# scrose/SVDSolver

Measured on AMD Instinct MI355X. Metric: GFLOP/s for two-stage bidiag reduction, N×N fp64, 1/2/4/8 MI355X, higher is better.
Workload: dtype f64; 1 GPU; stream of independent two-stage bidiagonal reductions 8192x8192 f64, band 32, stage 2 = reference window geometry (compat); n=8192, band=32, global_batch=10, parallelism=replicas1, pipeline=stage 2 of matrix i on a second HIP stream beside stage 1 of matrix i+1, stage2_cus=32, lanes=10, stage2_streams=5, hw_queues=19

## Files before the change

### svdsolver_amd/csrc/brd_s2win.h

```cpp
#pragma once

namespace brd {

template <typename T>
struct S2Ring {
    T *d;
    int P;
    int R;
    unsigned magic;
    __device__ __forceinline__ int slot(int r) const { return fast_mod(r, R, magic); }
    __device__ __forceinline__ T *row(int r) const { return d + slot(r) * P + 31 - r; }
};

template <typename T>
struct S2Fix {
    T sig;
    T alpha;
    T tau;
    T x31;
    T xl;
};

__device__ __forceinline__ double s2_readlane(double v, int l) {
    return __hiloint2double(__builtin_amdgcn_readlane(__double2hiint(v), l),
                            __builtin_amdgcn_readlane(__double2loint(v), l));
}
__device__ __forceinline__ float s2_readlane(float v, int l) {
    return __int_as_float(__builtin_amdgcn_readlane(__float_as_int(v), l));
}

template <typename T>
struct S2Sums {
    T q0, q1, q2, q3, g0, g1, g2, g3;
};
template <typename T>
__device__ __forceinline__ void s2_pin(S2Sums<T> &u) {
    if constexpr (sizeof(T) == 4)
        asm volatile("" : "+v"(u.q0), "+v"(u.q1), "+v"(u.q2), "+v"(u.q3), "+v"(u.g0), "+v"(u.g1), "+v"(u.g2), "+v"(u.g3));
}
template <typename T, int N>
__device__ __forceinline__ S2Sums<T> s2_sums(const T (&a)[N], const T (&x)[N]) {
    static_assert(N == 32, "b = 32 windows");
    S2Sums<T> u{x[0] * x[0], (T)0, (T)0, (T)0, (T)0, (T)0, (T)0, (T)0};
#pragma unroll
    for (int j = 1; j < N - 1; j += 4) {
        u.q1 = fma(x[j], x[j], u.q1);
        u.g1 = fma(a[j], x[j], u.g1);
        if (j + 1 < N - 1) { u.q2 = fma(x[j + 1], x[j + 1], u.q2); u.g2 = fma(a[j + 1], x[j + 1], u.g2); }
        if (j + 2 < N - 1) { u.q3 = fma(x[j + 2], x[j + 2], u.q3); u.g3 = fma(a[j + 2], x[j + 2], u.g3); }
        if (j + 3 < N - 1) { u.q0 = fma(x[j + 3], x[j + 3], u.q0); u.g0 = fma(a[j + 3], x[j + 3], u.g0); }
    }
    return u;
}
template <typename T, int N>
__device__ __forceinline__ T s2_apply(T (&a)[N], const T (&x)[N], S2Sums<T> u, S2Fix<T> &f) {
    u.q0 = fma(x[N - 1], x[N - 1], u.q0);
    const T qq = (u.q0 + u.q1) + (u.q2 + u.q3);
    const T sigp = (u.g0 + u.g1) + (u.g2 + u.g3);
    const T sig = fma(a[N - 1], x[N - 1], sigp);
    const T rn = rsq_nr(qq);
    const T nrm = qq * rn;
    const T sgn = x[0] >= (T)0 ? (T)-1 : (T)1;
    const T u1 = fma(-sgn, nrm, x[0]);
    const T alpha = rcp_nr(u1);
    const T tau = -sgn * u1 * rn;
    const T dot = fma(alpha, sig, a[0]);
    const T tda = (tau * dot) * alpha;
    a[0] = fma(-tau, dot, a[0]);
#pragma unroll
    for (int j = 1; j < N; ++j) a[j] = fma(-tda, x[j], a[j]);
    f.alpha = alpha;
    f.tau = tau;
    f.x31 = x[N - 1];
    return sigp;
}
template <typename T, int N>
__device__ __forceinline__ T s2_refl(T (&a)[N], const T (&x)[N], S2Fix<T> &f) {
    return s2_apply<T, N>(a, x, s2_sums<T, N>(a, x), f);
}

template <typename T, int N>
__device__ __forceinline__ void s2_fixup(T (&a)[N], T (&x)[N], const S2Fix<T> &f, T corner, int lane) {
    const T a0 = x[N - 1];
    const T dot = fma(f.alpha, fma(corner, f.x31, f.sig), a0);
    const T tda = (f.tau * dot) * f.alpha;
    const T p = fma(-f.tau, dot, a0);
    if (lane < 32) a[N - 1] = lane == 0 ? p : fma(-tda, f.xl, a[N - 1]);
    x[N - 1] = p;
}

struct S2Pub {
    int *prog, *front;
    int prog_v, front_v;
    __device__ __forceinline__ void publish(int lane) const {
        asm volatile("" ::: "memory");
        if (lane == 0) {
            __hip_atomic_store(front, front_v, __ATOMIC_RELAXED, __HIP_MEMORY_SCOPE_WORKGROUP);
            __hip_atomic_store(prog, prog_v, __ATOMIC_RELAXED, __HIP_MEMORY_SCOPE_WORKGROUP);
        }
    }
};

template <typename T>
__device__ __forceinline__ void s2_fixup1(T &a31, T &x31, const S2Fix<T> &f, T corner, int lane) {
    const T dot = fma(f.alpha, fma(corner, f.x31, f.sig), x31);
    const T tda = (f.tau * dot) * f.alpha;
    const T p = fma(-f.tau, dot, x31);
    if (lane < 32) a31 = lane == 0 ? p : fma(-tda, f.xl, a31);
    x31 = p;
}

template <typename T, bool FULL, bool LAG2>
__device__ __forceinline__ void s2_right_w1(const S2Ring<T> &rg, int i1, int j1, int nr, int nc, int lane,
                                            bool fix, const S2Fix<T> &fi, bool defer, S2Fix<T> &fo,
                                            const S2Pub &pub) {
    constexpr int N = 32;
    const bool rok = FULL || lane < nr;
    const T *px = rg.row(i1) + j1;
    T *pa = rg.row(i1 + (rok ? lane : 0)) + j1;
    T a[N], x[N];
#pragma unroll
    for (int j = 0; j < N; ++j) {
        const bool cok = FULL || j < nc;
        x[j] = cok ? px[j] : (T)0;
        a[j] = (cok && rok) ? pa[j] : (T)0;
    }
    if (LAG2) fo.xl = px[lane & 31];
    const T corner = LAG2 ? rg.row(i1 + 31)[j1 + 31] : (T)0;
    S2Sums<T> u = s2_sums<T, N>(a, x);
    s2_pin(u);
    if (LAG2 && fix) {
        s2_fixup1<T>(a[N - 1], x[N - 1], fi, corner, lane);
        if (lane < 32) pa[N - 1] = a[N - 1];
        pub.publish(lane);
    }
    const T sigp = s2_apply<T, N>(a, x, u, fo);
    if (LAG2 && defer) {
        fo.sig = s2_readlane(sigp, 63);
        if ((lane & 31) == 31) fo.xl = x[N - 1];
    }
    if (rok && !(LAG2 && defer && lane == 63)) {
#pragma unroll
        for (int j = 0; j < N; ++j)
            if (FULL || j < nc) pa[j] = a[j];
    }
}

template <typename T, bool FULL, bool LAG2>
__device__ __forceinline__ void s2_left_w1(const S2Ring<T> &rg, int i1, int j1, int nr, int nc, int lane,
                                           bool fix, const S2Fix<T> &fi, bool defer, S2Fix<T> &fo,
                                           const S2Pub &pub) {
    constexpr int N = 32;
    const bool cok = FULL || lane < nc;
    const int q = cok ? lane : 0;
    const int s0 = rg.slot(i1);
    T a[N], x[N];
    if (LAG2) fo.xl = rg.row(i1 + (lane & 31))[j1];
    auto finish = [&](T *e31, T corner, auto store) {
        S2Sums<T> u = s2_sums<T, N>(a, x);
        s2_pin(u);
        if (LAG2 && fix) {
            s2_fixup1<T>(a[N - 1], x[N - 1], fi, corner, lane);
            if (lane < 32) *e31 = a[N - 1];
            pub.publish(lane);
        }
        const T sigp = s2_apply<T, N>(a, x, u, fo);
        if (LAG2 && defer) {
            fo.sig = s2_readlane(sigp, 63);
            if ((lane & 31) == 31) fo.xl = x[N - 1];
        }
        if (cok && !(LAG2 && defer && lane == 63)) store();
    };
    if (s0 + N <= rg.R) {
        T *bx = rg.d + s0 * rg.P + 31 + (j1 - i1);
#pragma unroll
        for (int j = 0; j < N; ++j) {
            const bool rk = FULL || j < nr;
            x[j] = rk ? bx[j * (rg.P - 1)] : (T)0;
            a[j] = (rk && cok) ? bx[j * (rg.P - 1) + q] : (T)0;
        }
        T *b31 = bx + (N - 1) * (rg.P - 1);
        finish(b31 + q, LAG2 ? b31[31] : (T)0, [&]() {
#pragma unroll
            for (int j = 0; j < N; ++j)
                if (FULL || j < nr) bx[j * (rg.P - 1) + q] = a[j];
        });
    } else {
        T *rows[N];
        int s = s0;
#pragma unroll
        for (int j = 0; j < N; ++j) {
            rows[j] = rg.d + s * rg.P + 31 + (j1 - i1) - j;
            s = s + 1 == rg.R ? 0 : s + 1;
            const bool rk = FULL || j < nr;
            x[j] = rk ? rows[j][0] : (T)0;
            a[j] = (rk && cok) ? rows[j][q] : (T)0;
        }
        finish(rows[N - 1] + q, LAG2 ? rows[N - 1][31] : (T)0, [&]() {
#pragma unroll
            for (int j = 0; j < N; ++j)
                if (FULL || j < nr) rows[j][q] = a[j];
        });
    }
}


}
```

### svdsolver_amd/csrc/brd_stage2.hip

```cpp
#include "brd_internal.h"

#include <algorithm>
#include <cstdlib>

namespace brd {

template <typename T>
__device__ __forceinline__ T ld_c(const T *p) {
    return __hip_atomic_load(p, __ATOMIC_RELAXED, __HIP_MEMORY_SCOPE_AGENT);
}
template <typename T>
__device__ __forceinline__ void st_c(T *p, T v) {
    __hip_atomic_store(p, v, __ATOMIC_RELAXED, __HIP_MEMORY_SCOPE_AGENT);
}

__device__ __forceinline__ void wave_sync2() {
    __builtin_amdgcn_fence(__ATOMIC_RELEASE, "wavefront");
    __builtin_amdgcn_wave_barrier();
    __builtin_amdgcn_fence(__ATOMIC_ACQUIRE, "wavefront");
}

template <typename T>
struct Refl {
    T alpha;
    T tau;
};

template <typename T, bool EXACT>
__device__ __forceinline__ Refl<T> refl_regs(const T (&x)[32], int L) {
    T acc = (T)0;
    double s;
    T nrm;
    if constexpr (EXACT) {
#pragma clang fp contract(off)
#pragma unroll
        for (int r = 0; r < 32; ++r)
            if (r < L) acc = acc + x[r] * x[r];
        nrm = (T)sqrt((double)acc);
        s = -copysign(1.0, (double)x[0]);
    } else {
        T acc1 = (T)0;
#pragma unroll
        for (int r = 0; r < 32; r += 2) {
            if (r < L) acc = fma(x[r], x[r], acc);
            if (r + 1 < L) acc1 = fma(x[r + 1], x[r + 1], acc1);
        }
        nrm = sqrt(acc + acc1);
        s = x[0] >= (T)0 ? -1.0 : 1.0;
    }
    const double u1 = (double)x[0] - s * (double)nrm;
    Refl<T> h;
    h.alpha = (T)(1. / u1);
    h.tau = (T)(-s * u1 / (double)nrm);
    return h;
}

template <typename T, bool EXACT>
struct WaveLds {
    T w[64];
    T h[2];
};
template <typename T>
struct WaveLds<T, true> {
    T w[64];
    T h[2];
    T x[64];
    T H[32 * 33];
    T buf[64 * 33];
};

template <typename T>
struct HbmAcc {
    T *A;
    long lda;
    __device__ __forceinline__ T *row(int r) const { return A + (long)r * lda; }
    __device__ __forceinline__ T ld(const T *p) const { return ld_c(p); }
    __device__ __forceinline__ void st(T *p, T v) const { st_c(p, v); }
};
__device__ __forceinline__ int fast_mod(int r, int R, unsigned magic) {
    int s = r - (int)__umulhi((unsigned)r, magic) * R;
    return s >= R ? s - R : s;
}

template <typename T>
struct RingAcc {
    T *d;
// ... 570 lines not shown
struct SweepFlags {
    int prog[12];
    int front[12];
    int loaded;
    int freed;
    int avail;
    int wturn;
    int wclaim;
    int wpub;
};

#ifdef BRD_S2TRACE
constexpr int kTrB0 = 600, kTrNB = 4, kTrTasks = 600, kTrPub = 1024;
struct S2Trace {
    unsigned long long task[kTrNB][12][kTrTasks][4];
    unsigned long long pub[kTrNB][8][kTrPub][2];
    int npub[kTrNB][8];
    unsigned long long bundle[kTrNB][4];
    unsigned long long wr[kTrNB][256][8];
};
__device__ S2Trace g_s2tr;
#define TRB(beta) ((beta) >= kTrB0 && (beta) < kTrB0 + kTrNB)
#define TRT(beta, w, t, k)                                                                      \
    do {                                                                                        \
        if (TRB(beta) && (t) < kTrTasks && lane == 0)                                           \
            g_s2tr.task[(beta) - kTrB0][w][t][k] = __builtin_amdgcn_s_memrealtime();            \
    } while (0)
#define TRP(beta, kind, val)                                                                    \
    do {                                                                                        \
        if (TRB(beta) && lane == 0) {                                                           \
            const int q_ = g_s2tr.npub[(beta) - kTrB0][kind]++;                                 \
            if (q_ < kTrPub) {                                                                  \
                g_s2tr.pub[(beta) - kTrB0][kind][q_][0] = __builtin_amdgcn_s_memrealtime();     \
                g_s2tr.pub[(beta) - kTrB0][kind][q_][1] = (val);                                \
            }                                                                                   \
        }                                                                                       \
    } while (0)
#define TRW(beta, q, k)                                                                         \
    do {                                                                                        \
        if (TRB(beta) && (q) < 256 && lane == 0)                                                \
            g_s2tr.wr[(beta) - kTrB0][q][k] = __builtin_amdgcn_s_memrealtime();                 \
    } while (0)
#else
#define TRT(beta, w, t, k) do {} while (0)
#define TRP(beta, kind, val) do {} while (0)
#define TRW(beta, q, k) do {} while (0)
#endif

template <typename T> constexpr int sweeps_max_threads() { return sizeof(T) == 8 ? 512 : 768; }

__device__ __forceinline__ int lds_ld(const int *p) {
    return __hip_atomic_load(p, __ATOMIC_RELAXED, __HIP_MEMORY_SCOPE_WORKGROUP);
}
__device__ __forceinline__ void lds_st(int *p, int v) {
    __hip_atomic_store(p, v, __ATOMIC_RELAXED, __HIP_MEMORY_SCOPE_WORKGROUP);
}

struct SweepStages {
    int nst;
    int B[5];
    int G[4];
};
__device__ __forceinline__ int sweeps_next(const SweepStages &st, int w, int beta, int nbundles) {
    int k = 0;
    while (k + 1 < st.nst && beta >= st.B[k + 1]) ++k;
    int nx = beta + st.G[k];
    while (k + 1 < st.nst && nx >= st.B[k + 1]) {
        ++k;
        if (w >= st.G[k]) return nbundles;
        const int b0 = st.B[k];
        nx = b0 + (((w - b0) % st.G[k]) + st.G[k]) % st.G[k];
    }
    return nx;
}
__device__ __forceinline__ int sweeps_first(const SweepStages &st, int w, int nbundles) {
    for (int k = 0; k < st.nst; ++k) {
        if (w >= st.G[k]) return nbundles;
        const int b0 = st.B[k];
        const int c = b0 + (((w - b0) % st.G[k]) + st.G[k]) % st.G[k];
        if (c < st.B[k + 1]) return c;
    }
    return nbundles;
}
template <typename T, int WR>
__global__ void __launch_bounds__(sweeps_max_threads<T>())
k_sweeps(T *A, int n, long lda, int sigma, int S, int R, unsigned magic, int *rows_done, int *err, SweepStages st)
{
    constexpr int b = 32;
    extern __shared__ __align__(16) unsigned char smem[];
    const int P = ring_pitch<T>(b);
    T *ring = (T *)smem;
    const size_t ring_bytes = ((size_t)R * P * sizeof(T) + 15) & ~(size_t)15;
    SweepFlags *F = (SweepFlags *)(smem + ring_bytes);
    const int wave = __builtin_amdgcn_readfirstlane(threadIdx.x >> 6), lane = threadIdx.x & 63;
    const S2Ring<T> rg{ring, P, R, magic};
    const int nbundles = (n - 1 + S - 1) / S;

    for (int beta = sweeps_first(st, (int)blockIdx.x, nbundles); beta < nbundles;
         beta = sweeps_next(st, (int)blockIdx.x, beta, nbundles)) {
        const int i0 = beta * S;
        const int nsw = min(S, n - 1 - i0);
        if (threadIdx.x < 12) {
            F->prog[threadIdx.x] = 0;
            F->front[threadIdx.x] = (int)threadIdx.x < nsw ? i0 + (int)threadIdx.x : n;
        }
        if (threadIdx.x == 0) {
            F->loaded = i0; F->freed = i0; F->avail = 0;
            F->wturn = 0; F->wclaim = i0; F->wpub = i0;
        }
#ifdef BRD_S2TRACE
        if (threadIdx.x == 0 && TRB(beta)) {
            g_s2tr.bundle[beta - kTrB0][0] = __builtin_amdgcn_s_memrealtime();
            g_s2tr.bundle[beta - kTrB0][2] = blockIdx.x;
            g_s2tr.bundle[beta - kTrB0][3] = __builtin_amdgcn_s_getreg((20 << 0) | (0 << 6) | (3 << 11));
        }
#endif
        __syncthreads();

        if (wave < nsw) {
            const int i = i0 + wave;
            SweepIter it;
            it.init(n, n, b, i, sigma);
            const int prev_ntask = wave > 0 ? sweep_ntask(n, n, b, i - 1, sigma) : 0;
            S2Fix<T> fx{(T)0, (T)0, (T)0, (T)0, (T)0};
            bool pend = false;
            for (int t = 0; t < it.ntask; ++t) {
                bool right;
                const Win w = it.task(t, right);
                const int nr = w.i2 - w.i1, nc = w.j2 - w.j1;
                const bool live = nr > 0 && nc > 0;
                const bool full = live && (right ? (nr == 2 * b && nc == b) : (nr == b && nc == 2 * b));
                const bool defer = kS2Lag2 && full && it.next_at_least(t, b);
                int spins = 0;
                TRT(beta, wave, t, 0);
                if (wave > 0) {
                    const int need = min(t + (defer ? 4 - BRD_S2_DEFER_LAG2 : 4), prev_ntask);
                    while (lds_ld(&F->prog[wave - 1]) < need) {
                        __builtin_amdgcn_s_sleep(0);
                        if (++spins > kSpinLimit) { if (lane == 0) st_c(err, 12); break; }
                    }
                }
                TRT(beta, wave, t, 1);
                if (live) {
                    while (lds_ld(&F->loaded) < w.i2) {
                        __builtin_amdgcn_s_sleep(0);
                        if (++spins > kSpinLimit) { if (lane == 0) st_c(err, 13); break; }
                    }
                    TRT(beta, wave, t, 2);
                    asm volatile("" ::: "memory");
                    const S2Pub pub{&F->prog[wave], &F->front[wave], t, w.i1};
                    S2Fix<T> fo;
                    if (right) {
                        if (full) s2_right_w1<T, true, kS2Lag2>(rg, w.i1, w.j1, nr, nc, lane, pend, fx, defer, fo, pub);
                        else      s2_right_w1<T, false, kS2Lag2>(rg, w.i1, w.j1, nr, nc, lane, pend, fx, defer, fo, pub);
                    } else {
                        if (full) s2_left_w1<T, true, kS2Lag2>(rg, w.i1, w.j1, nr, nc, lane, pend, fx, defer, fo, pub);
                        else      s2_left_w1<T, false, kS2Lag2>(rg, w.i1, w.j1, nr, nc, lane, pend, fx, defer, fo, pub);
                    }
                    if (defer) fx = fo;
                    asm volatile("" ::: "memory");
                }
                pend = defer;
                TRT(beta, wave, t, 3);
                if (lane == 0) {
                    lds_st(&F->front[wave], it.next_top(t));
                    if (!defer) lds_st(&F->prog[wave], t + 1);
                }
            }
        } else if (wave == S) {
            const int row_q = P * (int)sizeof(T) / 16;
            const bool ql = lane < row_q;
            const unsigned row_bytes = (unsigned)(P * (int)sizeof(T));
            const unsigned ring_lds = (unsigned)(uintptr_t)ring;
            const unsigned ring_end = ring_lds + (unsigned)R * row_bytes;
            const int dma_hi = (int)(((long)(n - 1) * lda + n + (b - 1) - P) / (lda + 1));
            int ra = i0, rl = i0, spins = 0;
            unsigned dst = ring_lds + (unsigned)rg.slot(i0) * row_bytes;
            const char *src = (const char *)(A + (long)i0 * lda + i0 - (b - 1)) + 16 * lane;
            const long rstep = (lda + 1) * (long)sizeof(T);
            const bool dma_lane = lane < row_q;
            while (rl < n) {
                const int av = lds_ld(&F->avail);
                const int fr = lds_ld(&F->freed);
                const int lim = __builtin_amdgcn_readfirstlane(min(min(av, fr + R), min(n, rl + kFly)));
                bool moved = false;
                if (ra < lim) {
                    if (ra >= 1 && ra <= dma_hi) {
                        const int k = min(lim, dma_hi + 1) - ra;
                        if (dma_lane) {
                            const char *p = src;
                            unsigned d = dst;
                            for (int q = 0; q < k; ++q) {
                                dma16_sc1(p, d);
                                p += rstep;
                                d += row_bytes;
                                if (d == ring_end) d = ring_lds;
                            }
                        }
                        src += (long)k * rstep;
                        dst += (unsigned)k * row_bytes;
                        if (dst >= ring_end) dst -= ring_end - ring_lds;
                        ra += k;
                        moved = true;
                        TRP(beta, 5, ra);
                        TRP(beta, 7, (av <= fr + R ? 0 : 1) + (lim == rl + kFly ? 2 : 0));
                    } else if (ra == rl) {
                        load_edge_row<T>(A, lda, n, b, ra, (T *)((char *)ring + (dst - ring_lds)), row_q, lane);
                        asm volatile("s_waitcnt vmcnt(0) lgkmcnt(0)" ::: "memory");
                        ++ra;
                        rl = ra;
                        src += rstep;
                        dst += row_bytes;
                        if (dst == ring_end) dst = ring_lds;
                        if (lane == 0) lds_st(&F->loaded, rl);
                        moved = true;
                    }
                }
                if (ra > rl) {
                    const int keep = max(0, ra - rl - kChunk);
                    wait_vmcnt(keep);
                    rl = ra - keep;
                    if (lane == 0) lds_st(&F->loaded, rl);
                    TRP(beta, 0, rl);
                    spins = 0;
                } else if (BRD_S2_REGLOAD && !moved && ra < av && fr + R <= ra && ra >= 1 && ra <= dma_hi) {
                    const int k = __builtin_amdgcn_readfirstlane(min(min(kRG<T>, av - ra), dma_hi + 1 - ra));
                    u32x4 g[kRG<T>];
                    {
                        const __amdgpu_buffer_rsrc_t rs = __builtin_amdgcn_make_buffer_rsrc(
                            (void *)(A + (long)ra * lda + ra - (b - 1)), (short)0, 0x7fffffff, 0x00020000);
                        const int vo = 16 * (ql ? lane : 0);
#pragma unroll
                        for (int kk = 0; kk < kRG<T>; ++kk)
                            g[kk] = __builtin_amdgcn_raw_buffer_load_b128(rs, vo, (unsigned)((kk < k ? kk : 0) * rstep), 16);
                    }
                    const int sl0 = (int)((dst - ring_lds) / row_bytes);
                    int fl = fr + R;
#pragma unroll
                    for (int kk = 0; kk < kRG<T>; ++kk) {
                        if (kk < k) {
                            const int r = ra + kk;
                            if (r >= fl) {
                                if (kk > 0 && lane == 0) lds_st(&F->loaded, r);
                                int f2 = __builtin_amdgcn_readfirstlane(lds_ld(&F->freed));
                                while (f2 + R <= r) {
                                    __builtin_amdgcn_s_sleep(0);
                                    if (++spins > kSpinLimit) { if (lane == 0) st_c(err, 14); break; }
                                    f2 = __builtin_amdgcn_readfirstlane(lds_ld(&F->freed));
                                }
                                fl = f2 + R;
                            }
                            const int sl = sl0 + kk >= R ? sl0 + kk - R : sl0 + kk;
                            if (ql) *((u32x4 *)(ring + sl * P) + lane) = g[kk];
                        }
                    }
                    ra += k;
                    rl = ra;
                    src += (long)k * rstep;
                    dst += (unsigned)k * row_bytes;
                    if (dst >= ring_end) dst -= ring_end - ring_lds;
                    if (lane == 0) lds_st(&F->loaded, rl);
                    TRP(beta, 0, rl);
                    spins = 0;
                } else if (!moved) {
                    __builtin_amdgcn_s_sleep(0);
                    if (++spins > kSpinLimit) { if (lane == 0) st_c(err, 14); break; }
                }
            }
            asm volatile("s_waitcnt vmcnt(0)" ::: "memory");
        } else if (wave == S + 1 + kSweepWriters) {
            if (beta == 0) {
                if (lane == 0) lds_st(&F->avail, n);
            } else {
                const int *done_prev = rows_done + beta - 1;
                int av = 0, spins = 0;
                while (av < n) {
                    const int v = __builtin_amdgcn_readfirstlane(ld_c(done_prev));
                    if (v != av) {
                        av = v;
                        if (lane == 0) lds_st(&F->avail, v);
                        TRP(beta, 2, v);
                        spins = 0;
                    } else {
                        __builtin_amdgcn_s_sleep(1);
                        if (++spins > kSpinLimit) { if (lane == 0) st_c(err, 16); break; }
                    }
                }
            }
        } else if (wave > S && wave <= S + kSweepWriters) {
            const int wi = wave - S - 1;
            const int row_q = P * (int)sizeof(T) / 16;
            const long gstep = (lda + 1) * (long)sizeof(T);
            for (int q = wi;; q += kSweepWriters) {
                int spins = 0;
                while (lds_ld(&F->wturn) != q) {
                    __builtin_amdgcn_s_sleep(0);
                    if (++spins > kSpinLimit) { if (lane == 0) st_c(err, 15); break; }
                }
                const int wb = __builtin_amdgcn_readfirstlane(lds_ld(&F->wclaim));
                if (wb >= n) {
                    if (lane == 0) lds_st(&F->wturn, q + 1);
                    break;
                }
                int wt = wb;
                spins = 0;
                for (;;) {
                    int fmin = n;
                    for (int s = 0; s < nsw; ++s) fmin = min(fmin, lds_ld(&F->front[s]));
                    wt = __builtin_amdgcn_readfirstlane(min(min(fmin, lds_ld(&F->loaded)), wb + WR));
                    if (wt > wb) break;
                    __builtin_amdgcn_s_sleep(0);
                    if (++spins > kSpinLimit) { if (lane == 0) st_c(err, 15); break; }
                }
                if (wt <= wb) break;
                if (lane == 0) {
                    lds_st(&F->wclaim, wt);
                    lds_st(&F->wturn, q + 1);
                }
                TRP(beta, 3, wb);
                TRW(beta, q, 0);
                const int k = wt - wb;
                constexpr int kH = WR / 2;
                const int sl0 = rg.slot(wb);
                const unsigned rstride = (unsigned)gstep;
                for (int r0 = 0; r0 < k; r0 += kH) {
                    const int kh = min(kH, k - r0);
                    const int sl = sl0 + r0 >= R ? sl0 + r0 - R : sl0 + r0;
                    const int rb = wb + r0;
                    const bool fast = kh == kH && sl + kH <= R && rb >= b - 1 && rb + kH - 1 - (b - 1) + P <= n;
                    if (fast) {
                        u32x4 v[kH];
                        const u32x4 *srow = (const u32x4 *)(ring + sl * P) + (lane < row_q ? lane : 0);
#pragma unroll
                        for (int rr = 0; rr < kH; ++rr) v[rr] = srow[rr * (P / kEpp<T>)];
                        asm volatile("s_waitcnt lgkmcnt(0)" ::: "memory");
                        TRW(beta, q, 1 + 3 * (r0 / kH));
                        spins = 0;
                        while (lds_ld(&F->freed) != rb) {
                            __builtin_amdgcn_s_sleep(0);
                            if (++spins > kSpinLimit) { if (lane == 0) st_c(err, 15); break; }
                        }
                        if (lane == 0) lds_st(&F->freed, rb + kH);
                        TRP(beta, 6, rb + kH);
                        TRW(beta, q, 2 + 3 * (r0 / kH));
                        if (lane < row_q) {
                            const __amdgpu_buffer_rsrc_t rs = __builtin_amdgcn_make_buffer_rsrc(
                                (void *)(A + (long)rb * lda + rb - (b - 1)), (short)0, 0x7fffffff, 0x00020000);
#pragma unroll
                            for (int rr = 0; rr < kH; ++rr)
                                __builtin_amdgcn_raw_buffer_store_b128(v[rr], rs, 16 * lane, rr * rstride, 16);
                        }
                        TRW(beta, q, 3 + 3 * (r0 / kH));
                    } else {
                        for (int rr = 0; rr < kh; ++rr) {
                            const int r = rb + rr;
                            const int sk = sl + rr >= R ? sl + rr - R : sl + rr;
                            const u32x4 vr = ((const u32x4 *)(ring + sk * P))[lane < row_q ? lane : 0];
                            asm volatile("s_waitcnt lgkmcnt(0)" ::: "memory");
                            if (lane < row_q) {
                                if (r >= b - 1 && r - (b - 1) + P <= n) {
                                    st16_sc1((void *)((const char *)(A + (long)r * lda + r - (b - 1)) + 16 * lane), vr);
                                } else {
                                    T *ge = A + (long)r * lda + r - (b - 1) + lane * kEpp<T>;
                                    const int cc0 = r - (b - 1) + lane * kEpp<T>;
                                    T e[kEpp<T>];
                                    __builtin_memcpy(e, &vr, 16);
#pragma unroll
                                    for (int kk = 0; kk < kEpp<T>; ++kk)
                                        if (cc0 + kk >= 0 && cc0 + kk < n) st_c(ge + kk, e[kk]);
                                }
                            }
                        }
                        spins = 0;
                        while (lds_ld(&F->freed) != rb) {
                            __builtin_amdgcn_s_sleep(0);
                            if (++spins > kSpinLimit) { if (lane == 0) st_c(err, 15); break; }
                        }
                        if (lane == 0) lds_st(&F->freed, rb + kh);
                        TRP(beta, 6, rb + kh);
                    }
                }
                TRP(beta, 4, wt);
                asm volatile("s_waitcnt vmcnt(0)" ::: "memory");
                TRW(beta, q, 7);
                spins = 0;
                while (lds_ld(&F->wpub) != wb) {
                    __builtin_amdgcn_s_sleep(0);
                    if (++spins > kSpinLimit) { if (lane == 0) st_c(err, 15); break; }
                }
                if (lane == 0) {
                    st_c(rows_done + beta, wt);
                    lds_st(&F->wpub, wt);
                }
                TRP(beta, 1, wt);
            }
        }
        __syncthreads();
#ifdef BRD_S2TRACE
        if (threadIdx.x == 0 && TRB(beta)) g_s2tr.bundle[beta - kTrB0][1] = __builtin_amdgcn_s_memrealtime();
#endif
    }
}

#ifdef BRD_S2TRACE
extern "C" int brd_dbg_s2trace(void *dst, size_t bytes, int reset) {
    if (reset) {
        static S2Trace z;
        return (int)hipMemcpyToSymbol(HIP_SYMBOL(g_s2tr), &z, sizeof(S2Trace));
    }
    return (int)hipMemcpyFromSymbol(dst, HIP_SYMBOL(g_s2tr), bytes < sizeof(S2Trace) ? bytes : sizeof(S2Trace));
}
#endif

template <typename T>
__global__ void k_extract(const T *A, int n, long lda, T *d, T *e)
{
    const int i = blockIdx.x * blockDim.x + threadIdx.x;
    if (i < n) d[i] = A[(long)i * lda + i];
    if (i < n - 1) e[i] = A[(long)i * lda + i + 1];
}

int ring_min_rows(int b, int S) { return ((3 * (S - 1)) / 2 + 2) * b + S + 8; }

template <typename T, bool EXACT>
static size_t bundle_lds_bytes(int b, int S, int R) {
    const size_t ring = ((size_t)R * ring_pitch<T>(b) * sizeof(T) + 15) & ~(size_t)15;
    return ring + (size_t)S * sizeof(WaveLds<T, EXACT>) + sizeof(BundleFlags);
}

template <typename T, bool EXACT>
static bool bundle_plan(int n, int b, int &S, int &R) {
    const size_t budget = 160 * 1024 - 512;
    static const char *senv = getenv("BRD_S2_SWEEPS");
    int smax = EXACT ? 2 : bundle_max_threads<T>() / 64 - 3;
    if (senv && atoi(senv) > 0) smax = std::min(smax, atoi(senv));
    const bool forced = senv && atoi(senv) > 0;
    for (int slack : {forced ? 8 : 16, 8}) {
        for (S = std::min(smax, std::max(1, n - 1)); S >= 1; --S) {
            const int rmin = ring_min_rows(b, S) + slack;
            if (bundle_lds_bytes<T, EXACT>(b, S, rmin) <= budget) {
                static const char *renv = getenv("BRD_S2_RING");
                const int rcap = renv && atoi(renv) > 0 ? std::max(rmin, atoi(renv)) : 1 << 30;
                R = rmin;
                while (R < n + 1 && R + 8 <= rcap && bundle_lds_bytes<T, EXACT>(b, S, R + 8) <= budget) R += 8;
                return true;
            }
        }
    }
    return false;
}

constexpr int kSweepSlack = 40;
template <typename T>
static size_t sweeps_lds_bytes(int R, int S) {
    (void)S;
    return (((size_t)R * ring_pitch<T>(32) * sizeof(T) + 15) & ~(size_t)15) + ((sizeof(SweepFlags) + 15) & ~(size_t)15);
}
template <typename T>
static bool sweeps_plan(int n, int &S, int &R) {
    const size_t budget = 160 * 1024;
    static const char *senv = getenv("BRD_S2_SWEEPS");
    int smax = sweeps_max_threads<T>() / 64 - 2 - kSweepWriters;
    if (smax > 12) smax = 12;
    if (senv && atoi(senv) > 0) smax = std::min(smax, atoi(senv));
    for (S = std::min(smax, std::max(1, n - 1)); S >= 1; --S) {
        const int rmin = ring_min_rows(32, S) + kSweepSlack;
        if (sweeps_lds_bytes<T>(rmin, S) <= budget) {
            R = rmin;
            while (R < n + 1 && sweeps_lds_bytes<T>(R + 1, S) <= budget) ++R;
            return true;
        }
    }
    return false;
}

static int coresident_limit(const void *fn, int threads, size_t lds) {
    int per_cu = 0, dev = 0, cus = 0;
    if (hipOccupancyMaxActiveBlocksPerMultiprocessor(&per_cu, fn, threads, lds) != hipSuccess) return 0;
    hipGetDevice(&dev);
    if (hipDeviceGetAttribute(&cus, hipDeviceAttributeMultiprocessorCount, dev) != hipSuccess) return 0;
    return per_cu * cus;
}

static SweepStages sweep_stages(int n, int S, int nbundles, int grid) {
    SweepStages st{};
    st.nst = 1;
    st.B[0] = 0;
    st.G[0] = grid;
    st.B[1] = nbundles;
    const char *e = getenv("BRD_S2_STAGES");
    if (e && atoi(e) == 0) return st;
    int g = grid;
    for (int beta = 0; beta < nbundles && st.nst < 4; ++beta) {
        const double alive = (double)(n - beta * S) / (64.0 * S) + 1.0;
        const int half = g / 2;
        if (half >= kStageMin && g % 2 == 0 && beta >= st.B[st.nst - 1] + g &&
            alive * kStageMargin + kStageSpare <= half) {
            st.B[st.nst] = beta;
            st.G[st.nst] = half;
            ++st.nst;
            g = half;
        }
    }
    st.B[st.nst] = nbundles;
    return st;
}

template <typename T>
hipError_t launch_band2bd(T *A, int n, long lda, int b, bool exact_order, bool sigma_geom, int *prog, int *err,
                          int nwaves, hipStream_t s)
{
    hipError_t e = hipMemsetAsync(prog, 0, sizeof(int) * (size_t)(n + 1), s);
    if (e != hipSuccess) return e;
    const int sg = sigma_geom ? 1 : 0;
    static const char *sel = getenv("BRD_S2_SCHEDULE");
    const bool pipe = sel && sel[0] == 'p';
    int S = 0, R = 0;
    const bool fast32 = !exact_order && b == 32;
    if (!pipe && fast32 && n >= 64 && sweeps_plan<T>(n, S, R)) {
        const int nbundles = (n - 1 + S - 1) / S;
        const dim3 block(64 * (S + 2 + kSweepWriters));
        const unsigned magic = (unsigned)((0x100000000ull + R - 1) / R);
        const bool w32 = sweep_rows_for(n) == 32;
        const void *fn = w32 ? (const void *)k_sweeps<T, 32> : (const void *)k_sweeps<T, 16>;
        const size_t lds = sweeps_lds_bytes<T>(R, S);
        e = hipFuncSetAttribute(fn, hipFuncAttributeMaxDynamicSharedMemorySize, (int)lds);
        if (e != hipSuccess) return e;
        const int cap = coresident_limit(fn, (int)block.x, lds);
        if (cap < 1) return hipErrorInvalidConfiguration;
        const int grid = std::max(1, std::min(std::min(nwaves, cap), nbundles));
        const SweepStages st = sweep_stages(n, S, nbundles, grid);
        if (w32) hipLaunchKernelGGL((k_sweeps<T, 32>), dim3(grid), block, lds, s, A, n, lda, sg, S, R, magic, prog, err, st);
        else     hipLaunchKernelGGL((k_sweeps<T, 16>), dim3(grid), block, lds, s, A, n, lda, sg, S, R, magic, prog, err, st);
        return hipGetLastError();
    }
    const bool ok = exact_order ? bundle_plan<T, true>(n, b, S, R) : bundle_plan<T, false>(n, b, S, R);
    if (!pipe && ok && n >= 64) {
        const int nbundles = (n - 1 + S - 1) / S;
        const dim3 block(64 * (S + 3));
        const unsigned magic = (unsigned)((0x100000000ull + R - 1) / R);
        const void *fn = exact_order ? (const void *)k_band2bd_bundle<T, true> : (const void *)k_band2bd_bundle<T, false>;
        const size_t lds = exact_order ? bundle_lds_bytes<T, true>(b, S, R) : bundle_lds_bytes<T, false>(b, S, R);
        e = hipFuncSetAttribute(fn, hipFuncAttributeMaxDynamicSharedMemorySize, (int)lds);
        if (e != hipSuccess) return e;
        const int cap = coresident_limit(fn, (int)block.x, lds);
        if (cap < 1) return hipErrorInvalidConfiguration;
        const int grid = std::max(1, std::min(std::min(nwaves, cap), nbundles));
        if (exact_order)
            hipLaunchKernelGGL((k_band2bd_bundle<T, true>), dim3(grid), block, lds, s, A, n, lda, b, sg, S, R, magic, prog, err);
        else
            hipLaunchKernelGGL((k_band2bd_bundle<T, false>), dim3(grid), block, lds, s, A, n, lda, b, sg, S, R, magic, prog, err);
        return hipGetLastError();
    }
    const void *pfn = exact_order ? (const void *)k_band2bd_pipe<T, true> : (const void *)k_band2bd_pipe<T, false>;
    const int cap = coresident_limit(pfn, 64, 0);
    if (cap < 1) return hipErrorInvalidConfiguration;
    const int grid = std::max(1, std::min(std::min(nwaves, cap), n - 1));
    if (exact_order)
        hipLaunchKernelGGL((k_band2bd_pipe<T, true>), dim3(grid), dim3(64), 0, s, A, n, n, lda, b, sg, prog, err);
    else
        hipLaunchKernelGGL((k_band2bd_pipe<T, false>), dim3(grid), dim3(64), 0, s, A, n, n, lda, b, sg, prog, err);
    return hipGetLastError();
}

template <typename T>
hipError_t launch_extract_bidiag(const T *A, int n, long lda, T *d, T *e, hipStream_t s)
{
    hipLaunchKernelGGL((k_extract<T>), dim3((n + 255) / 256), dim3(256), 0, s, A, n, lda, d, e);
    return hipGetLastError();
}

template hipError_t launch_band2bd<double>(double *, int, long, int, bool, bool, int *, int *, int, hipStream_t);
template hipError_t launch_band2bd<float>(float *, int, long, int, bool, bool, int *, int *, int, hipStream_t);
template hipError_t launch_extract_bidiag<double>(const double *, int, long, double *, double *, hipStream_t);
template hipError_t launch_extract_bidiag<float>(const float *, int, long, float *, float *, hipStream_t);

}
```

Before: 27710 GFLOP/s.

## Store stage-2 sweep ring in LDS with per-phase narrow row pitch

Adds a phase-dependent narrow row layout for the fp64 stage-2 LDS ring. Each row stores only the columns its phase in the 32-row group actually touches, so the same LDS budget holds more rows. The loader, writer and left-window code are rewritten to use per-phase offsets and widths, and the sweep index is made a compile-time constant per wave. The layout is on by default for fp64 and caps sweeps per bundle at 4 (default 3) instead of up to 12, so parallelism within a bundle drops. It also adds more complex index arithmetic.

After: 19450 GFLOP/s. -29.8%, worse.

```diff
diff --git a/svdsolver_amd/csrc/brd_s2_ring.h b/svdsolver_amd/csrc/brd_s2_ring.h
--- /dev/null
+++ b/svdsolver_amd/csrc/brd_s2_ring.h
@@ -0,0 +1,81 @@
+#pragma once
+
+#include <cstddef>
+
+#ifndef BRD_HD
+#ifdef __HIPCC__
+#define BRD_HD __host__ __device__
+#else
+#define BRD_HD
+#endif
+#endif
+
+namespace brd {
+namespace s2ring {
+
+constexpr int kB = 32;
+constexpr int kMaxSweeps = 4;
+constexpr int kWidePhases = kMaxSweeps - 1;
+constexpr int kWideW = 96;
+constexpr int kWideLo = -31;
+constexpr int kNarrowW = 68;
+
+BRD_HD constexpr int ph_width(int p) { return p < kWidePhases ? kWideW : kNarrowW; }
+BRD_HD constexpr int ph_skew(int p) { return p < 16 ? 1 : 0; }
+BRD_HD constexpr int ph_dlo(int p) { return p < kWidePhases ? kWideLo : -p - ph_skew(p); }
+BRD_HD constexpr int ph_off(int p) {
+    return p < kWidePhases ? kWideW * p : kWideW * kWidePhases + kNarrowW * (p - kWidePhases) + 2 * (p >> 3);
+}
+BRD_HD constexpr int ph_zero(int p) { return ph_off(p) - ph_dlo(p); }
+constexpr int kGroupElems = ph_off(31) + kNarrowW;
+
+BRD_HD constexpr int idx_off(int idx) { return (idx >> 5) * kGroupElems + ph_off(idx & 31); }
+
+BRD_HD inline int ring_index(int i0, int r, int R) {
+    int u = (r - i0 - 1) % R;
+    return u < 0 ? u + R : u;
+}
+
+struct Row {
+    int off;
+    int c0;
+    int w;
+};
+BRD_HD inline Row row_map(int i0, int r, int R) {
+    const int idx = ring_index(i0, r, R);
+    const int p = idx & 31;
+    return Row{idx_off(idx), r + ph_dlo(p), ph_width(p)};
+}
+
+BRD_HD constexpr int left_carry(int sw, int j) { return (sw + j) >> 5; }
+BRD_HD constexpr int left_off(int sw, int j) { return ph_zero((sw + j) & 31) - j; }
+
+BRD_HD constexpr int ring_min_rows(int b, int S) { return ((3 * (S - 1)) / 2 + 2) * b + S + 8; }
+constexpr int kSweepSlack = 40;
+
+BRD_HD constexpr size_t ring_bytes(int groups, size_t esz) { return (size_t)groups * kGroupElems * esz; }
+
+constexpr int kDefaultSweeps = 3;
+struct Plan {
+    bool ok;
+    int S, G, R;
+    size_t bytes;
+};
+BRD_HD inline Plan plan(int n, int s_req, size_t esz, size_t budget, size_t tail) {
+    Plan pl{false, 0, 0, 0, 0};
+    int S = s_req > 0 ? s_req : kDefaultSweeps;
+    if (S > kMaxSweeps) S = kMaxSweeps;
+    if (S > n - 1) S = n - 1 > 1 ? n - 1 : 1;
+    if (budget < tail) return pl;
+    const int G = (int)((budget - tail) / ring_bytes(1, esz));
+    for (; S >= 1; --S) {
+        if (32 * G >= ring_min_rows(kB, S) + kSweepSlack) {
+            pl = Plan{true, S, G, 32 * G, ring_bytes(G, esz) + tail};
+            return pl;
+        }
+    }
+    return pl;
+}
+
+}
+}
diff --git a/svdsolver_amd/csrc/brd_s2win.h b/svdsolver_amd/csrc/brd_s2win.h
--- a/svdsolver_amd/csrc/brd_s2win.h
+++ b/svdsolver_amd/csrc/brd_s2win.h
@@ -1,15 +1,32 @@
 #pragma once
 
+#include "brd_s2_ring.h"
+
 namespace brd {
 
 template <typename T>
 struct S2Ring {
+    static constexpr bool kNarrow = false;
     T *d;
     int P;
     int R;
     unsigned magic;
     __device__ __forceinline__ int slot(int r) const { return fast_mod(r, R, magic); }
     __device__ __forceinline__ T *row(int r) const { return d + slot(r) * P + 31 - r; }
+};
+
+template <typename T>
+struct S2RingN {
+    static constexpr bool kNarrow = true;
+    T *d;
+    int R;
+    unsigned magic;
+    int org;
+    __device__ __forceinline__ int index(int r) const { return fast_mod(r - org, R, magic); }
+    __device__ __forceinline__ T *row(int r) const {
+        const int idx = index(r);
+        return d + ((idx >> 5) * s2ring::kGroupElems + s2ring::ph_zero(idx & 31)) - r;
+    }
 };
 
 template <typename T>
@@ -110,8 +127,8 @@
     x31 = p;
 }
 
-template <typename T, bool FULL, bool LAG2>
-__device__ __forceinline__ void s2_right_w1(const S2Ring<T> &rg, int i1, int j1, int nr, int nc, int lane,
+template <typename T, bool FULL, bool LAG2, typename RG>
+__device__ __forceinline__ void s2_right_w1(const RG &rg, int i1, int j1, int nr, int nc, int lane,
                                             bool fix, const S2Fix<T> &fi, bool defer, S2Fix<T> &fo,
                                             const S2Pub &pub) {
     constexpr int N = 32;
@@ -146,14 +163,13 @@
     }
 }
 
-template <typename T, bool FULL, bool LAG2>
-__device__ __forceinline__ void s2_left_w1(const S2Ring<T> &rg, int i1, int j1, int nr, int nc, int lane,
+template <typename T, bool FULL, bool LAG2, int SW, typename RG>
+__device__ __forceinline__ void s2_left_w1(const RG &rg, int i1, int j1, int nr, int nc, int lane,
                                            bool fix, const S2Fix<T> &fi, bool defer, S2Fix<T> &fo,
                                            const S2Pub &pub) {
     constexpr int N = 32;
     const bool cok = FULL || lane < nc;
     const int q = cok ? lane : 0;
-    const int s0 = rg.slot(i1);
     T a[N], x[N];
     if (LAG2) fo.xl = rg.row(i1 + (lane & 31))[j1];
     auto finish = [&](T *e31, T corner, auto store) {
@@ -171,7 +187,24 @@
         }
         if (cok && !(LAG2 && defer && lane == 63)) store();
     };
-    if (s0 + N <= rg.R) {
+    if constexpr (RG::kNarrow) {
+        const int g0 = __builtin_amdgcn_readfirstlane(rg.index(i1) >> 5);
+        const int g1 = g0 + 1 == (rg.R >> 5) ? 0 : g0 + 1;
+        T *const bg[2] = {rg.d + g0 * s2ring::kGroupElems + (j1 - i1), rg.d + g1 * s2ring::kGroupElems + (j1 - i1)};
+#pragma unroll
+        for (int j = 0; j < N; ++j) {
+            const bool rk = FULL || j < nr;
+            T *bj = bg[s2ring::left_carry(SW, j)] + s2ring::left_off(SW, j);
+            x[j] = rk ? bj[0] : (T)0;
+            a[j] = (rk && cok) ? bj[q] : (T)0;
+        }
+        T *b31 = bg[s2ring::left_carry(SW, N - 1)] + s2ring::left_off(SW, N - 1);
+        finish(b31 + q, LAG2 ? b31[31] : (T)0, [&]() {
+#pragma unroll
+            for (int j = 0; j < N; ++j)
+                if (FULL || j < nr) bg[s2ring::left_carry(SW, j)][s2ring::left_off(SW, j) + q] = a[j];
+        });
+    } else if (const int s0 = rg.slot(i1); s0 + N <= rg.R) {
         T *bx = rg.d + s0 * rg.P + 31 + (j1 - i1);
 #pragma unroll
         for (int j = 0; j < N; ++j) {
@@ -187,7 +220,7 @@
         });
     } else {
         T *rows[N];
-        int s = s0;
+        int s = rg.slot(i1);
 #pragma unroll
         for (int j = 0; j < N; ++j) {
             rows[j] = rg.d + s * rg.P + 31 + (j1 - i1) - j;
diff --git a/svdsolver_amd/csrc/brd_stage2.hip b/svdsolver_amd/csrc/brd_stage2.hip
--- a/svdsolver_amd/csrc/brd_stage2.hip
+++ b/svdsolver_amd/csrc/brd_stage2.hip
@@ -2,6 +2,7 @@
 
 #include <algorithm>
 #include <cstdlib>
+#include <type_traits>
 
 namespace brd {
 
@@ -738,24 +739,45 @@
     }
     return nbundles;
 }
-template <typename T, int WR>
+template <typename T, bool NARROW> struct SweepRing { typedef S2Ring<T> type; };
+template <typename T> struct SweepRing<T, true> { typedef S2RingN<T> type; };
+template <typename T>
+__device__ __forceinline__ void load_edge_row_n(const T *A, long lda, int n, int r, int c0, T *dst, int npc, int lane) {
+    if (lane < npc) {
+        T e[kEpp<T>];
+#pragma unroll
+        for (int k = 0; k < kEpp<T>; ++k) {
+            const int c = c0 + lane * kEpp<T> + k;
+            e[k] = (c >= 0 && c < n) ? ld_c(A + (long)r * lda + c) : (T)0;
+        }
+        u32x4 v;
+        __builtin_memcpy(&v, e, 16);
+        *(u32x4 *)(dst + lane * kEpp<T>) = v;
+    }
+}
+
+template <typename T, int WR, bool NARROW>
 __global__ void __launch_bounds__(sweeps_max_threads<T>())
 k_sweeps(T *A, int n, long lda, int sigma, int S, int R, unsigned magic, int *rows_done, int *err, SweepStages st)
 {
     constexpr int b = 32;
+    static_assert(!NARROW || sizeof(T) == 8, "the row-phase pitch is fp64 only");
     extern __shared__ __align__(16) unsigned char smem[];
     const int P = ring_pitch<T>(b);
     T *ring = (T *)smem;
-    const size_t ring_bytes = ((size_t)R * P * sizeof(T) + 15) & ~(size_t)15;
+    const size_t ring_bytes = NARROW ? s2ring::ring_bytes(R >> 5, sizeof(T))
+                                     : (((size_t)R * P * sizeof(T) + 15) & ~(size_t)15);
     SweepFlags *F = (SweepFlags *)(smem + ring_bytes);
     const int wave = __builtin_amdgcn_readfirstlane(threadIdx.x >> 6), lane = threadIdx.x & 63;
-    const S2Ring<T> rg{ring, P, R, magic};
     const int nbundles = (n - 1 + S - 1) / S;
 
     for (int beta = sweeps_first(st, (int)blockIdx.x, nbundles); beta < nbundles;
          beta = sweeps_next(st, (int)blockIdx.x, beta, nbundles)) {
         const int i0 = beta * S;
         const int nsw = min(S, n - 1 - i0);
+        typename SweepRing<T, NARROW>::type rg;
+        if constexpr (NARROW) rg = S2RingN<T>{ring, R, magic, i0 + 1 - R};
+        else                  rg = S2Ring<T>{ring, P, R, magic};
         if (threadIdx.x < 12) {
             F->prog[threadIdx.x] = 0;
             F->front[threadIdx.x] = (int)threadIdx.x < nsw ? i0 + (int)threadIdx.x : n;
@@ -810,8 +832,22 @@
                         if (full) s2_right_w1<T, true, kS2Lag2>(rg, w.i1, w.j1, nr, nc, lane, pend, fx, defer, fo, pub);
                         else      s2_right_w1<T, false, kS2Lag2>(rg, w.i1, w.j1, nr, nc, lane, pend, fx, defer, fo, pub);
                     } else {
-                        if (full) s2_left_w1<T, true, kS2Lag2>(rg, w.i1, w.j1, nr, nc, lane, pend, fx, defer, fo, pub);
-                        else      s2_left_w1<T, false, kS2Lag2>(rg, w.i1, w.j1, nr, nc, lane, pend, fx, defer, fo, pub);
+                        auto left = [&](auto swc) {
+                            constexpr int SW = decltype(swc)::value;
+                            if (full) s2_left_w1<T, true, kS2Lag2, SW>(rg, w.i1, w.j1, nr, nc, lane, pend, fx, defer, fo, pub);
+                            else      s2_left_w1<T, false, kS2Lag2, SW>(rg, w.i1, w.j1, nr, nc, lane, pend, fx, defer, fo, pub);
+                        };
+                        if constexpr (NARROW) {
+                            static_assert(s2ring::kMaxSweeps == 4, "one case per sweep of a bundle");
+                            switch (wave) {
+                                case 0: left(std::integral_constant<int, 0>{}); break;
+                                case 1: left(std::integral_constant<int, 1>{}); break;
+                                case 2: left(std::integral_constant<int, 2>{}); break;
+                                default: left(std::integral_constant<int, 3>{}); break;
+                            }
+                        } else {
+                            left(std::integral_constant<int, 0>{});
+                        }
                     }
                     if (defer) fx = fo;
                     asm volatile("" ::: "memory");
@@ -824,6 +860,107 @@
                 }
             }
         } else if (wave == S) {
+            if constexpr (NARROW) {
+            constexpr int kE = kEpp<T>;
+            const unsigned ring_lds = (unsigned)(uintptr_t)ring;
+            const int dma_hi = (int)(((long)(n - 1) * lda + n - (s2ring::kWideLo + s2ring::kWideW)) / (lda + 1));
+            int ra = i0, rl = i0, spins = 0;
+            int ia = __builtin_amdgcn_readfirstlane(rg.index(i0));
+            const char *src = (const char *)(A + (long)i0 * lda + i0) + 16 * lane;
+            const long rstep = (lda + 1) * (long)sizeof(T);
+            while (rl < n) {
+                const int av = lds_ld(&F->avail);
+                const int fr = lds_ld(&F->freed);
+                const int lim = __builtin_amdgcn_readfirstlane(min(min(av, fr + R), min(n, rl + kFly)));
+                bool moved = false;
+                if (ra < lim) {
+                    if (ra >= 1 && ra <= dma_hi) {
+                        const int k = min(lim, dma_hi + 1) - ra;
+                        const char *p = src;
+                        int ix = ia;
+                        for (int q = 0; q < k; ++q) {
+                            const int ph = ix & 31;
+                            const unsigned d = __builtin_amdgcn_readfirstlane(
+                                ring_lds + (unsigned)(s2ring::idx_off(ix) * (int)sizeof(T)));
+                            if (lane < s2ring::ph_width(ph) / kE) dma16_sc1(p + s2ring::ph_dlo(ph) * (int)sizeof(T), d);
+                            p += rstep;
+                            ix = ix + 1 == R ? 0 : ix + 1;
+                        }
+                        src += (long)k * rstep;
+                        ia = ia + k >= R ? ia + k - R : ia + k;
+                        ra += k;
+                        moved = true;
+                        TRP(beta, 5, ra);
+                        TRP(beta, 7, (av <= fr + R ? 0 : 1) + (lim == rl + kFly ? 2 : 0));
+                    } else if (ra == rl) {
+                        const int ph = ia & 31;
+                        load_edge_row_n<T>(A, lda, n, ra, ra + s2ring::ph_dlo(ph), ring + s2ring::idx_off(ia),
+                                           s2ring::ph_width(ph) / kE, lane);
+                        asm volatile("s_waitcnt vmcnt(0) lgkmcnt(0)" ::: "memory");
+                        ++ra;
+                        rl = ra;
+                        src += rstep;
+                        ia = ia + 1 == R ? 0 : ia + 1;
+                        if (lane == 0) lds_st(&F->loaded, rl);
+                        moved = true;
+                    }
+                }
+                if (ra > rl) {
+                    const int keep = max(0, ra - rl - kChunk);
+                    wait_vmcnt(keep);
+                    rl = ra - keep;
+                    if (lane == 0) lds_st(&F->loaded, rl);
+                    TRP(beta, 0, rl);
+                    spins = 0;
+                } else if (BRD_S2_REGLOAD && !moved && ra < av && fr + R <= ra && ra >= 1 && ra <= dma_hi) {
+                    const int k = __builtin_amdgcn_readfirstlane(min(min(kRG<T>, av - ra), dma_hi + 1 - ra));
+                    u32x4 g[kRG<T>];
+                    {
+                        const __amdgpu_buffer_rsrc_t rs = __builtin_amdgcn_make_buffer_rsrc(
+                            (void *)(A + (long)ra * lda + ra + s2ring::kWideLo), (short)0, 0x7fffffff, 0x00020000);
+#pragma unroll
+                        for (int kk = 0; kk < kRG<T>; ++kk) {
+                            const int kq = kk < k ? kk : 0;
+                            const int ix = ia + kq >= R ? ia + kq - R : ia + kq;
+                            const int ph = ix & 31;
+                            const int vo = 16 * (lane < s2ring::ph_width(ph) / kE ? lane : 0);
+                            g[kk] = __builtin_amdgcn_raw_buffer_load_b128(
+                                rs, vo, (unsigned)(kq * rstep + (s2ring::ph_dlo(ph) - s2ring::kWideLo) * (int)sizeof(T)), 16);
+                        }
+                    }
+                    int fl = fr + R;
+#pragma unroll
+                    for (int kk = 0; kk < kRG<T>; ++kk) {
+                        if (kk < k) {
+                            const int r = ra + kk;
+                            if (r >= fl) {
+                                if (kk > 0 && lane == 0) lds_st(&F->loaded, r);
+                                int f2 = __builtin_amdgcn_readfirstlane(lds_ld(&F->freed));
+                                while (f2 + R <= r) {
+                                    __builtin_amdgcn_s_sleep(0);
+                                    if (++spins > kSpinLimit) { if (lane == 0) st_c(err, 14); break; }
+                                    f2 = __builtin_amdgcn_readfirstlane(lds_ld(&F->freed));
+                                }
+                                fl = f2 + R;
+                            }
+                            const int ix = ia + kk >= R ? ia + kk - R : ia + kk;
+                            if (lane < s2ring::ph_width(ix & 31) / kE) *((u32x4 *)(ring + s2ring::idx_off(ix)) + lane) = g[kk];
+                        }
+                    }
+                    ra += k;
+                    rl = ra;
+                    src += (long)k * rstep;
+                    ia = ia + k >= R ? ia + k - R : ia + k;
+                    if (lane == 0) lds_st(&F->loaded, rl);
+                    TRP(beta, 0, rl);
+                    spins = 0;
+                } else if (!moved) {
+                    __builtin_amdgcn_s_sleep(0);
+                    if (++spins > kSpinLimit) { if (lane == 0) st_c(err, 14); break; }
+                }
+            }
+            asm volatile("s_waitcnt vmcnt(0)" ::: "memory");
+            } else {
             const int row_q = P * (int)sizeof(T) / 16;
             const bool ql = lane < row_q;
             const unsigned row_bytes = (unsigned)(P * (int)sizeof(T));
@@ -924,6 +1061,7 @@
                 }
             }
             asm volatile("s_waitcnt vmcnt(0)" ::: "memory");
+            }
         } else if (wave == S + 1 + kSweepWriters) {
             if (beta == 0) {
                 if (lane == 0) lds_st(&F->avail, n);
@@ -977,8 +1115,82 @@
                 TRW(beta, q, 0);
                 const int k = wt - wb;
                 constexpr int kH = WR / 2;
+                const unsigned rstride = (unsigned)gstep;
+                if constexpr (NARROW) {
+                constexpr int kE = kEpp<T>;
+                const int ix0 = __builtin_amdgcn_readfirstlane(rg.index(wb));
+                for (int r0 = 0; r0 < k; r0 += kH) {
+                    const int kh = min(kH, k - r0);
+                    const int ixb = ix0 + r0 >= R ? ix0 + r0 - R : ix0 + r0;
+                    const int rb = wb + r0;
+                    const bool fast = kh == kH && rb >= -s2ring::kWideLo &&
+                                      rb + kH - 1 + s2ring::kWideLo + s2ring::kWideW <= n;
+                    if (fast) {
+                        u32x4 v[kH];
+#pragma unroll
+                        for (int rr = 0; rr < kH; ++rr) {
+                            const int ix = ixb + rr >= R ? ixb + rr - R : ixb + rr;
+                            const int npc = s2ring::ph_width(ix & 31) / kE;
+                            v[rr] = ((const u32x4 *)(ring + s2ring::idx_off(ix)))[lane < npc ? lane : 0];
+                        }
+                        asm volatile("s_waitcnt lgkmcnt(0)" ::: "memory");
+                        TRW(beta, q, 1 + 3 * (r0 / kH));
+                        spins = 0;
+                        while (lds_ld(&F->freed) != rb) {
+                            __builtin_amdgcn_s_sleep(0);
+                            if (++spins > kSpinLimit) { if (lane == 0) st_c(err, 15); break; }
+                        }
+                        if (lane == 0) lds_st(&F->freed, rb + kH);
+                        TRP(beta, 6, rb + kH);
+                        TRW(beta, q, 2 + 3 * (r0 / kH));
+                        {
+                            const __amdgpu_buffer_rsrc_t rs = __builtin_amdgcn_make_buffer_rsrc(
+                                (void *)(A + (long)rb * lda + rb + s2ring::kWideLo), (short)0, 0x7fffffff, 0x00020000);
+#pragma unroll
+                            for (int rr = 0; rr < kH; ++rr) {
+                                const int ix = ixb + rr >= R ? ixb + rr - R : ixb + rr;
+                                const int ph = ix & 31;
+                                if (lane < s2ring::ph_width(ph) / kE)
+                                    __builtin_amdgcn_raw_buffer_store_b128(
+                                        v[rr], rs, 16 * lane,
+                                        rr * rstride + (unsigned)((s2ring::ph_dlo(ph) - s2ring::kWideLo) * (int)sizeof(T)), 16);
+                            }
+                        }
+                        TRW(beta, q, 3 + 3 * (r0 / kH));
+                    } else {
+                        for (int rr = 0; rr < kh; ++rr) {
+                            const int r = rb + rr;
+                            const int ix = ixb + rr >= R ? ixb + rr - R : ixb + rr;
+                            const int ph = ix & 31;
+                            const int npc = s2ring::ph_width(ph) / kE;
+                            const int c0 = r + s2ring::ph_dlo(ph);
+                            const u32x4 vr = ((const u32x4 *)(ring + s2ring::idx_off(ix)))[lane < npc ? lane : 0];
+                            asm volatile("s_waitcnt lgkmcnt(0)" ::: "memory");
+                            if (lane < npc) {
+                                if (c0 >= 0 && c0 + npc * kE <= n) {
+                                    st16_sc1((void *)((const char *)(A + (long)r * lda + c0) + 16 * lane), vr);
+                                } else {
+                                    T *ge = A + (long)r * lda + c0 + lane * kE;
+                                    const int cc0 = c0 + lane * kE;
+                                    T e[kE];
+                                    __builtin_memcpy(e, &vr, 16);
+#pragma unroll
+                                    for (int kk = 0; kk < kE; ++kk)
+                                        if (cc0 + kk >= 0 && cc0 + kk < n) st_c(ge + kk, e[kk]);
+                                }
+                            }
+                        }
+                        spins = 0;
+                        while (lds_ld(&F->freed) != rb) {
+                            __builtin_amdgcn_s_sleep(0);
+                            if (++spins > kSpinLimit) { if (lane == 0) st_c(err, 15); break; }
+                        }
+                        if (lane == 0) lds_st(&F->freed, rb + kh);
+                        TRP(beta, 6, rb + kh);
+                    }
+                }
+                } else {
                 const int sl0 = rg.slot(wb);
-                const unsigned rstride = (unsigned)gstep;
                 for (int r0 = 0; r0 < k; r0 += kH) {
                     const int kh = min(kH, k - r0);
                     const int sl = sl0 + r0 >= R ? sl0 + r0 - R : sl0 + r0;
@@ -1036,6 +1248,7 @@
                         TRP(beta, 6, rb + kh);
                     }
                 }
+                }
                 TRP(beta, 4, wt);
                 asm volatile("s_waitcnt vmcnt(0)" ::: "memory");
                 TRW(beta, q, 7);
@@ -1076,7 +1289,7 @@
     if (i < n - 1) e[i] = A[(long)i * lda + i + 1];
 }
 
-int ring_min_rows(int b, int S) { return ((3 * (S - 1)) / 2 + 2) * b + S + 8; }
+using s2ring::ring_min_rows;
 
 template <typename T, bool EXACT>
 static size_t bundle_lds_bytes(int b, int S, int R) {
@@ -1106,24 +1319,41 @@
     return false;
 }
 
-constexpr int kSweepSlack = 40;
+using s2ring::kSweepSlack;
+constexpr bool kSweepPhasePitch = true;
+constexpr size_t kSweepFlagBytes = (sizeof(SweepFlags) + 15) & ~(size_t)15;
 template <typename T>
-static size_t sweeps_lds_bytes(int R, int S) {
+static size_t sweeps_lds_bytes(int R, int S, bool narrow) {
     (void)S;
-    return (((size_t)R * ring_pitch<T>(32) * sizeof(T) + 15) & ~(size_t)15) + ((sizeof(SweepFlags) + 15) & ~(size_t)15);
+    if (narrow) return s2ring::ring_bytes(R / 32, sizeof(T)) + kSweepFlagBytes;
+    return (((size_t)R * ring_pitch<T>(32) * sizeof(T) + 15) & ~(size_t)15) + kSweepFlagBytes;
 }
 template <typename T>
-static bool sweeps_plan(int n, int &S, int &R) {
+static bool sweeps_narrow() {
+    if (sizeof(T) != 8) return false;
+    const char *e = getenv("BRD_S2_PITCH");
+    if (e && e[0] == 'u') return false;
+    if (e && e[0] == 'p') return true;
+    return kSweepPhasePitch;
+}
+template <typename T>
+static bool sweeps_plan(int n, int &S, int &R, bool narrow) {
     const size_t budget = 160 * 1024;
-    static const char *senv = getenv("BRD_S2_SWEEPS");
+    const char *senv = getenv("BRD_S2_SWEEPS");
+    if (narrow) {
+        const s2ring::Plan pl = s2ring::plan(n, senv ? atoi(senv) : 0, sizeof(T), budget, kSweepFlagBytes);
+        S = pl.S;
+        R = pl.R;
+        return pl.ok && S + 2 + kSweepWriters <= sweeps_max_threads<T>() / 64;
+    }
     int smax = sweeps_max_threads<T>() / 64 - 2 - kSweepWriters;
     if (smax > 12) smax = 12;
     if (senv && atoi(senv) > 0) smax = std::min(smax, atoi(senv));
     for (S = std::min(smax, std::max(1, n - 1)); S >= 1; --S) {
         const int rmin = ring_min_rows(32, S) + kSweepSlack;
-        if (sweeps_lds_bytes<T>(rmin, S) <= budget) {
+        if (sweeps_lds_bytes<T>(rmin, S, false) <= budget) {
             R = rmin;
-            while (R < n + 1 && sweeps_lds_bytes<T>(R + 1, S) <= budget) ++R;
+            while (R < n + 1 && sweeps_lds_bytes<T>(R + 1, S, false) <= budget) ++R;
             return true;
         }
     }
@@ -1173,21 +1403,29 @@
     const bool pipe = sel && sel[0] == 'p';
     int S = 0, R = 0;
     const bool fast32 = !exact_order && b == 32;
-    if (!pipe && fast32 && n >= 64 && sweeps_plan<T>(n, S, R)) {
+    const bool narrow = sweeps_narrow<T>();
+    if (!pipe && fast32 && n >= 64 && sweeps_plan<T>(n, S, R, narrow)) {
         const int nbundles = (n - 1 + S - 1) / S;
         const dim3 block(64 * (S + 2 + kSweepWriters));
         const unsigned magic = (unsigned)((0x100000000ull + R - 1) / R);
         const bool w32 = sweep_rows_for(n) == 32;
-        const void *fn = w32 ? (const void *)k_sweeps<T, 32> : (const void *)k_sweeps<T, 16>;
-        const size_t lds = sweeps_lds_bytes<T>(R, S);
+        constexpr bool kN = sizeof(T) == 8;
+        const void *fn = narrow ? (w32 ? (const void *)k_sweeps<T, 32, kN> : (const void *)k_sweeps<T, 16, kN>)
+                                : (w32 ? (const void *)k_sweeps<T, 32, false> : (const void *)k_sweeps<T, 16, false>);
+        const size_t lds = sweeps_lds_bytes<T>(R, S, narrow);
         e = hipFuncSetAttribute(fn, hipFuncAttributeMaxDynamicSharedMemorySize, (int)lds);
         if (e != hipSuccess) return e;
         const int cap = coresident_limit(fn, (int)block.x, lds);
         if (cap < 1) return hipErrorInvalidConfiguration;
         const int grid = std::max(1, std::min(std::min(nwaves, cap), nbundles));
         const SweepStages st = sweep_stages(n, S, nbundles, grid);
-        if (w32) hipLaunchKernelGGL((k_sweeps<T, 32>), dim3(grid), block, lds, s, A, n, lda, sg, S, R, magic, prog, err, st);
-        else     hipLaunchKernelGGL((k_sweeps<T, 16>), dim3(grid), block, lds, s, A, n, lda, sg, S, R, magic, prog, err, st);
+        if (narrow) {
+            if (w32) hipLaunchKernelGGL((k_sweeps<T, 32, kN>), dim3(grid), block, lds, s, A, n, lda, sg, S, R, magic, prog, err, st);
+            else     hipLaunchKernelGGL((k_sweeps<T, 16, kN>), dim3(grid), block, lds, s, A, n, lda, sg, S, R, magic, prog, err, st);
+        } else {
+            if (w32) hipLaunchKernelGGL((k_sweeps<T, 32, false>), dim3(grid), block, lds, s, A, n, lda, sg, S, R, magic, prog, err, st);
+            else     hipLaunchKernelGGL((k_sweeps<T, 16, false>), dim3(grid), block, lds, s, A, n, lda, sg, S, R, magic, prog, err, st);
+        }
         return hipGetLastError();
     }
     const bool ok = exact_order ? bundle_plan<T, true>(n, b, S, R) : bundle_plan<T, false>(n, b, S, R);
```
